# Suaiba/Mammo-CLIP-Dissect

Hardware: AMD Instinct MI355X
Metric: probe images/sec dissected (763 concepts, all layers) (higher is better)
Workload: dtype f32; 1 GPU; configs[1]: M-Mammo-CLIP Dissect through the drop-in driver describe_broad_neurons.main(): Mammo-CLIP ViT-B/16 target+dissector (random init), weak: 10000 images per GPU, synthetic 224x224 images resident in HBM, 763 concepts, 12 layers x 768 neurons, soft_wpmi top_k=100; CSV + args.txt + activation cache files written inside the step; entry_point=mammo_clip_dissect_amd.concept_vit.describe_broad_neurons.main, images_per_gpu=10000, global_images=10000, batch=2500, parallelism=image-sharded dp1, activation_cache_written=True

## Files before the change

mammo-clip-dissect_amd/csrc/k_attn.hip:

```cpp
#include "mcd_common.h"
#include "../../include/mcd_text.h"
#include "../../include/mcd_clip.h"
#include "../../include/mcd_sentence.h"

namespace {

using f32x16 = __attribute__((ext_vector_type(16))) float;

constexpr int AT_D = 64;
constexpr int AT_MAX_T = 256;
constexpr int AT_LONG_MAX_T = 32768;
constexpr int AT_HALF = 32 * 256;
constexpr int AT_STAGE = 2 * AT_HALF;
constexpr int AT_NSTAGE = 4;
constexpr int AT_REL = 2 * AT_MAX_T + 32;

template <bool KEYLEN, bool CAUSAL = false, bool BIAS = false>
__device__ __forceinline__ void attn_block(const float* __restrict__ qkv, int T, int H, int64_t b, int h, int q0, int ncw,
                                           int L, float* __restrict__ out, const float* __restrict__ rel = nullptr) {
    __shared__ __attribute__((aligned(1024))) char at_lds[AT_NSTAGE * AT_STAGE];
    const float* rel_s = nullptr;
    if constexpr (BIAS) {
        __shared__ float at_rel[AT_REL];
        for (int i = threadIdx.x; i < AT_REL; i += blockDim.x) {
            const int d = i - (T - 1);
            at_rel[i] = d < L ? rel[max(d, 1 - L) + T - 1] * 1.44269504088896340736f : 0.f;
        }
        rel_s = at_rel;
        __syncthreads();
    }
    const int TK = KEYLEN ? L : T;
    const int ntile = (TK + 31) >> 5;
    const int64_t row_stride = (int64_t)3 * H * AT_D;
    const float* base = qkv + b * T * row_stride + (int64_t)h * AT_D;
    const int lane = threadIdx.x & 63;
    const int wave = __builtin_amdgcn_readfirstlane(threadIdx.x >> 6);
    const int ql = lane & 31, half = lane >> 5;
    const int q = q0 + wave * 32 + ql;

    if (wave == ncw) {
        auto stage = [&](int kt) {
            __amdgpu_buffer_rsrc_t rs = __builtin_amdgcn_make_buffer_rsrc((void*)(qkv + b * T * row_stride), 0,
                                                                            (int)(T * row_stride * 4), 0x00020000);
            char* dst = at_lds + (kt % AT_NSTAGE) * AT_STAGE;
            const int v_off = H * AT_D * 4;
#pragma unroll
            for (int p = 0; p < 8; ++p) {
                const int r = 4 * p + (lane >> 4);
                const int c = (lane & 15) ^ (r & 15);
                int key = kt * 32 + r;
                if (key >= TK) key = TK - 1;
                const unsigned off = (unsigned)(((int64_t)key * row_stride + (int64_t)(h + H) * AT_D + c * 4) * 4);
                __builtin_amdgcn_raw_ptr_buffer_load_lds(rs, (__attribute__((address_space(3))) void*)(dst + p * 1024), 16, off, 0, 0, 0);
                __builtin_amdgcn_raw_ptr_buffer_load_lds(rs, (__attribute__((address_space(3))) void*)(dst + AT_HALF + p * 1024), 16, off,
                                                         v_off, 0, 0);
            }
        };
        stage(0);
        if (ntile > 1) stage(1);
        for (int kt = 0; kt < ntile; kt += 2) {
            asm volatile("s_waitcnt vmcnt(0)" ::: "memory");
            __builtin_amdgcn_s_barrier();
            asm volatile("" ::: "memory");
            if (kt + 2 < ntile) stage(kt + 2);
            if (kt + 3 < ntile) stage(kt + 3);
        }
        return;
    }

    const float qs = 0.125f * 1.44269504088896340736f;
    float Qr[32];
    const float* qrow = base + (int64_t)(q < T ? q : T - 1) * row_stride + 4 * half;
    float4 qv[8];
#pragma unroll
    for (int j = 0; j < 8; ++j) qv[j] = *reinterpret_cast<const float4*>(qrow + 8 * j);
#pragma unroll
    for (int j = 0; j < 8; ++j) {
        const float4 t = qv[j];
        Qr[4 * j + 0] = t.x * qs;
        Qr[4 * j + 1] = t.y * qs;
        Qr[4 * j + 2] = t.z * qs;
        Qr[4 * j + 3] = t.w * qs;
    }

    const int kx = ql & 15;
    const int k_off = ql * 256;
    const int v_row = 4 * half * 256 + (ql & 3) * 4;
    const int va = (ql >> 2) ^ (half << 2);

    f32x16 o[2];
#pragma unroll
    for (int i = 0; i < 2; ++i)
#pragma unroll
        for (int r = 0; r < 16; ++r) o[i][r] = 0.f;
    float m = -INFINITY, l = 0.f;
    const int rel_q = T - 1 - (q < T ? q : T - 1) + 4 * half;

    const int ntile_w = CAUSAL ? min(ntile, (q0 >> 5) + wave + 1) : ntile;
    for (int kt = 0; kt < ntile_w; ++kt) {
        if ((kt & 1) == 0) __builtin_amdgcn_s_barrier();
        asm volatile("" ::: "memory");
        const char* kb = at_lds + (kt % AT_NSTAGE) * AT_STAGE;
        const char* vb = kb + AT_HALF;
        int kx_t = kx, va_t = va;
        asm volatile("" : "+v"(kx_t), "+v"(va_t));
        int v_off[4];
#pragma unroll
        for (int e = 0; e < 4; ++e) v_off[e] = v_row + ((va_t ^ e) << 4);

        f32x16 c;
#pragma unroll
        for (int r = 0; r < 16; ++r) c[r] = 0.f;
#pragma unroll
        for (int j = 0; j < 8; ++j) {
            const float4 ka = *reinterpret_cast<const float4*>(kb + k_off + (((2 * j + half) ^ kx_t) << 4));
            c = __builtin_amdgcn_mfma_f32_32x32x2f32(ka.x, Qr[4 * j + 0], c, 0, 0, 0);
            c = __builtin_amdgcn_mfma_f32_32x32x2f32(ka.y, Qr[4 * j + 1], c, 0, 0, 0);
            c = __builtin_amdgcn_mfma_f32_32x32x2f32(ka.z, Qr[4 * j + 2], c, 0, 0, 0);
            c = __builtin_amdgcn_mfma_f32_32x32x2f32(ka.w, Qr[4 * j + 3], c, 0, 0, 0);
        }
        if constexpr (BIAS) {
            const float* rb = rel_s + rel_q + kt * 32;
#pragma unroll
            for (int r = 0; r < 16; ++r) c[r] += rb[(r & 3) + 8 * (r >> 2)];
        }
        if constexpr (CAUSAL) {
            if (kt == ntile_w - 1) {
#pragma unroll
                for (int r = 0; r < 16; ++r)
                    if ((r & 3) + 8 * (r >> 2) + 4 * half > ql) c[r] = -INFINITY;
            }
        } else {
            const int nk = TK - kt * 32;
            if (nk < 32) {
#pragma unroll
                for (int r = 0; r < 16; ++r)
                    if ((r & 3) + 8 * (r >> 2) + 4 * half >= nk) c[r] = -INFINITY;
            }
        }
        float mt = c[0];
#pragma unroll
        for (int r = 1; r < 16; ++r) mt = fmaxf(mt, c[r]);
        mt = fmaxf(mt, __shfl_xor(mt, 32));
        const float m_new = fmaxf(m, mt);
        const float alpha = __builtin_amdgcn_exp2f(m - m_new);
        float ls = 0.f;
#pragma unroll
        for (int r = 0; r < 16; ++r) {
            c[r] = __builtin_amdgcn_exp2f(c[r] - m_new);
            ls += c[r];
        }
        l = l * alpha + ls;
        m = m_new;
#pragma unroll
        for (int i = 0; i < 2; ++i)
#pragma unroll
            for (int r = 0; r < 16; ++r) o[i][r] *= alpha;
        auto pv_step = [&](int r) {
            const int k0 = (r & 3) + 8 * (r >> 2);
            const char* vr = vb + k0 * 256 + v_off[r & 3];
            const float v0 = *reinterpret_cast<const float*>(vr + ((0 ^ (k0 & 8)) << 4));
            const float v1 = *reinterpret_cast<const float*>(vr + ((8 ^ (k0 & 8)) << 4));
            o[0] = __builtin_amdgcn_mfma_f32_32x32x2f32(v0, c[r], o[0], 0, 0, 0);
            o[1] = __builtin_amdgcn_mfma_f32_32x32x2f32(v1, c[r], o[1], 0, 0, 0);
        };
#pragma unroll
        for (int r = 0; r < 16; ++r) {
            if ((r & 3) == 0 && r) asm volatile("" ::: "memory");
            pv_step(r);
        }
    }

    l = l + __shfl_xor(l, 32);
    if (q < T) {
        const float inv = 1.0f / l;
        float* dst = out + (b * T + q) * (int64_t)H * AT_D + (int64_t)h * AT_D + 4 * half;
#pragma unroll
        for (int i = 0; i < 2; ++i)
#pragma unroll
            for (int g = 0; g < 4; ++g) {
                const float4 t = make_float4(o[i][4 * g + 0] * inv, o[i][4 * g + 1] * inv, o[i][4 * g + 2] * inv,
                                             o[i][4 * g + 3] * inv);
                *reinterpret_cast<float4*>(dst + 32 * i + 8 * g) = t;
            }
    }
    if constexpr (CAUSAL) {
        for (int kt = (ntile_w + 1) & ~1; kt < ntile; kt += 2) __builtin_amdgcn_s_barrier();
    }
}

__global__ __launch_bounds__(576, 4) void vit_attention_kernel(const float* __restrict__ qkv, int T, int H,
                                                                float* __restrict__ out) {
    const int ntile = (T + 31) >> 5;
    const int h = blockIdx.x;
    const int64_t b = blockIdx.y;
    attn_block<false>(qkv, T, H, b, h, 0, ntile, T, out);
}

__global__ __launch_bounds__(576, 4) void vit_attention_keylen_kernel(const float* __restrict__ qkv, int T, int H,
                                                                       const int32_t* __restrict__ lens,
                                                                       float* __restrict__ out) {
    const int ncw = (T + 31) >> 5;
    const int h = blockIdx.x;
    const int64_t b = blockIdx.y;
    int L = T;
    if (lens) L = min(max(lens[b], 1), T);
    attn_block<true>(qkv, T, H, b, h, 0, ncw, __builtin_amdgcn_readfirstlane(L), out);
}

__global__ __launch_bounds__(576, 4) void vit_attention_relbias_kernel(const float* __restrict__ qkv, int T, int H,
                                                                        const int32_t* __restrict__ lens,
                                                                        const float* __restrict__ rel,
                                                                        float* __restrict__ out) {
    const int ncw = (T + 31) >> 5;
    const int h = blockIdx.x;
    const int64_t b = blockIdx.y;
    int L = T;
    if (lens) L = min(max(lens[b], 1), T);
    attn_block<true, false, true>(qkv, T, H, b, h, 0, ncw, __builtin_amdgcn_readfirstlane(L), out,
                                  rel + (int64_t)h * (2 * T - 1));
}

__global__ __launch_bounds__(576, 4) void vit_attention_causal_kernel(const float* __restrict__ qkv, int T, int H,
                                                                       float* __restrict__ out) {
    const int ntile = (T + 31) >> 5;
    const int h = blockIdx.x;
    const int64_t b = blockIdx.y;
    attn_block<false, true>(qkv, T, H, b, h, 0, ntile, T, out);
}

__global__ __launch_bounds__(576, 4) void vit_attention_long_kernel(const float* __restrict__ qkv, int T, int H, int nqb,
                                                                     int npairs, int per_xcd, float* __restrict__ out) {
    const int pair = (int)(blockIdx.x & 7) * per_xcd + (int)(blockIdx.x >> 3);
    if (pair >= npairs) return;
    const int grp = pair / nqb;
    const int ncw = min(8, (T + 31) >> 5);
    attn_block<false>(qkv, T, H, grp / H, grp % H, (pair - grp * nqb) * 32 * ncw, ncw, T, out);
}

constexpr int AC_WAVES = 4;
constexpr int AC_U = 4;
constexpr int AC_SPLIT_T = 512;
constexpr int AC_MAX_T = 32768;

template <int CTRL>
__device__ __forceinline__ float ac_dpp_add(float x) {
    return x + __builtin_bit_cast(float, __builtin_amdgcn_update_dpp(0, __builtin_bit_cast(int, x), CTRL, 0xf, 0xf, true));
}

__device__ __forceinline__ float ac_row_sum(float x) {
    x = ac_dpp_add<0xB1>(x);
    x = ac_dpp_add<0x4E>(x);
    x = ac_dpp_add<0x141>(x);
    return ac_dpp_add<0x140>(x);
}

__global__ __launch_bounds__(64 * AC_WAVES) void vit_attention_cls_kernel(
    const float* __restrict__ q, int64_t q_img, const float* __restrict__ k, int64_t k_row, int64_t k_img,
    const float* __restrict__ v, int64_t v_row, int64_t v_img, int T, int H, int64_t npairs, int S, float* __restrict__ out) {
    __shared__ float4 st_acc[AC_WAVES * 4][16];
    __shared__ float st_m[AC_WAVES * 4], st_l[AC_WAVES * 4];
    const int lane = threadIdx.x & 63;
    const int wave = __builtin_amdgcn_readfirstlane(threadIdx.x >> 6);
    const int sub = lane & 15, g = lane >> 4;
    const int64_t pair = (int64_t)blockIdx.x * (AC_WAVES / S) + wave / S;
    const int slice = wave % S;
    const bool live = pair < npairs;

    float m = -1e30f, l = 0.f;
    float4 acc = make_float4(0.f, 0.f, 0.f, 0.f);
    if (live) {
        const int64_t b = pair / H;
        const int h = (int)(pair - b * H);
        const float qs = 0.125f * 1.44269504088896340736f;
        float4 qv = *reinterpret_cast<const float4*>(q + b * q_img + (int64_t)h * AT_D + 4 * sub);
        qv.x *= qs; qv.y *= qs; qv.z *= qs; qv.w *= qs;
        const int r0 = slice * 4 + g;
        const float* kp = k + b * k_img + (int64_t)r0 * k_row + (int64_t)h * AT_D + 4 * sub;
        const float* vp = v + b * v_img + (int64_t)r0 * v_row + (int64_t)h * AT_D + 4 * sub;
        const int64_t kstep = (int64_t)4 * S * k_row, vstep = (int64_t)4 * S * v_row;
        for (int rb = slice * 4; rb < T; rb += 4 * S * AC_U) {
            float4 kk[AC_U], vv[AC_U];
            bool ok[AC_U];
#pragma unroll
            for (int u = 0; u < AC_U; ++u) {
                ok[u] = rb + u * 4 * S + g < T;
                kk[u] = make_float4(0.f, 0.f, 0.f, 0.f);
                vv[u] = make_float4(0.f, 0.f, 0.f, 0.f);
                if (ok[u]) {
                    kk[u] = *reinterpret_cast<const float4*>(kp + u * kstep);
                    vv[u] = *reinterpret_cast<const float4*>(vp + u * vstep);
                }
            }
            kp += AC_U * kstep;
            vp += AC_U * vstep;
            float s[AC_U];
            float mt = m;
#pragma unroll
            for (int u = 0; u < AC_U; ++u) {
                const float d = fmaf(kk[u].w, qv.w, fmaf(kk[u].z, qv.z, fmaf(kk[u].y, qv.y, kk[u].x * qv.x)));
                const float r = ac_row_sum(d);
                s[u] = ok[u] ? r : -INFINITY;
                mt = fmaxf(mt, s[u]);
            }
            const float alpha = __builtin_amdgcn_exp2f(m - mt);
            m = mt;
            l *= alpha;
            acc.x *= alpha; acc.y *= alpha; acc.z *= alpha; acc.w *= alpha;
#pragma unroll
            for (int u = 0; u < AC_U; ++u) {
                const float p = __builtin_amdgcn_exp2f(s[u] - mt);
                l += p;
                acc.x = fmaf(p, vv[u].x, acc.x);
                acc.y = fmaf(p, vv[u].y, acc.y);
                acc.z = fmaf(p, vv[u].z, acc.z);
                acc.w = fmaf(p, vv[u].w, acc.w);
            }
        }
    }
    st_acc[wave * 4 + g][sub] = acc;
    if (sub == 0) {
        st_m[wave * 4 + g] = m;
        st_l[wave * 4 + g] = l;
    }
    __syncthreads();
    if (live && slice == 0) {
        const int s0 = wave * 4, ns = 4 * S;
        float mx = st_m[s0];
        for (int i = 1; i < ns; ++i) mx = fmaxf(mx, st_m[s0 + i]);
        float num = 0.f, den = 0.f;
        const float* accf = reinterpret_cast<const float*>(&st_acc[s0][0]);
        for (int i = 0; i < ns; ++i) {
            const float w = __builtin_amdgcn_exp2f(st_m[s0 + i] - mx);
            num = fmaf(accf[i * 64 + lane], w, num);
            den = fmaf(st_l[s0 + i], w, den);
        }
        out[pair * AT_D + lane] = num / den;
    }
}

}

extern "C" int mcd_vit_attention(const float* qkv, int64_t B, int64_t T, int64_t H, float* out, mcd_stream_t stream) {
    MCD_REQUIRE(qkv && out, MCD_E_ARG, "mcd_vit_attention: NULL pointer");
    MCD_REQUIRE(B >= 0 && T >= 1 && H >= 1, MCD_E_ARG, "mcd_vit_attention: bad shape B=%lld T=%lld H=%lld", (long long)B,
                (long long)T, (long long)H);
    MCD_REQUIRE(T <= AT_MAX_T, MCD_E_UNSUPPORTED, "mcd_vit_attention: T=%lld tokens, at most %d (one wave per 32 queries, 8 waves)",
                (long long)T, AT_MAX_T);
    MCD_REQUIRE(B <= 65535 && H <= 65535, MCD_E_UNSUPPORTED, "mcd_vit_attention: B and H must be <= 65535");
    MCD_REQUIRE(((uintptr_t)qkv) % 16 == 0 && ((uintptr_t)out) % 16 == 0, MCD_E_ARG,
                "mcd_vit_attention: qkv and out must be 16-byte aligned");
    if (B == 0) return MCD_OK;
    const int nwaves = (int)((T + 31) / 32) + 1;
    hipLaunchKernelGGL(vit_attention_kernel, dim3((unsigned)H, (unsigned)B), dim3(64 * nwaves), 0, (hipStream_t)stream, qkv,
                       (int)T, (int)H, out);
    MCD_LAUNCH_CHECK("vit_attention_kernel");
    return MCD_OK;
}

extern "C" int mcd_vit_attention_keylen(const float* qkv, int64_t B, int64_t T, int64_t H, const int32_t* lens, float* out,
                                        mcd_stream_t stream) {
    MCD_REQUIRE(qkv && out, MCD_E_ARG, "mcd_vit_attention_keylen: NULL pointer");
    MCD_REQUIRE(B >= 0 && T >= 1 && H >= 1, MCD_E_ARG, "mcd_vit_attention_keylen: bad shape B=%lld T=%lld H=%lld",
                (long long)B, (long long)T, (long long)H);
    MCD_REQUIRE(T <= AT_MAX_T, MCD_E_UNSUPPORTED,
                "mcd_vit_attention_keylen: T=%lld tokens, at most %d (one wave per 32 queries, 8 waves)", (long long)T, AT_MAX_T);
    MCD_REQUIRE(B <= 65535 && H <= 65535, MCD_E_UNSUPPORTED, "mcd_vit_attention_keylen: B and H must be <= 65535");
    MCD_REQUIRE(((uintptr_t)qkv) % 16 == 0 && ((uintptr_t)out) % 16 == 0 && ((uintptr_t)lens) % 4 == 0, MCD_E_ARG,
                "mcd_vit_attention_keylen: qkv and out must be 16-byte aligned, lens 4-byte aligned");
    if (B == 0) return MCD_OK;
    const int nwaves = (int)((T + 31) / 32) + 1;
    hipLaunchKernelGGL(vit_attention_keylen_kernel, dim3((unsigned)H, (unsigned)B), dim3(64 * nwaves), 0, (hipStream_t)stream,
                       qkv, (int)T, (int)H, lens, out);
    MCD_LAUNCH_CHECK("vit_attention_keylen_kernel");
    return MCD_OK;
}

extern "C" int mcd_vit_attention_relbias(const float* qkv, int64_t B, int64_t T, int64_t H, const int32_t* lens,
                                         const float* rel, float* out, mcd_stream_t stream) {
    MCD_REQUIRE(qkv && out, MCD_E_ARG, "mcd_vit_attention_relbias: NULL pointer");
    MCD_REQUIRE(B >= 0 && T >= 1 && H >= 1, MCD_E_ARG, "mcd_vit_attention_relbias: bad shape B=%lld T=%lld H=%lld",
                (long long)B, (long long)T, (long long)H);
    MCD_REQUIRE(T <= AT_MAX_T, MCD_E_UNSUPPORTED,
                "mcd_vit_attention_relbias: T=%lld tokens, at most %d (one wave per 32 queries, 8 waves)", (long long)T, AT_MAX_T);
    MCD_REQUIRE(B <= 65535 && H <= 65535, MCD_E_UNSUPPORTED, "mcd_vit_attention_relbias: B and H must be <= 65535");
    MCD_REQUIRE(((uintptr_t)qkv) % 16 == 0 && ((uintptr_t)out) % 16 == 0 && ((uintptr_t)lens) % 4 == 0 &&
                    ((uintptr_t)rel) % 16 == 0,
                MCD_E_ARG, "mcd_vit_attention_relbias: qkv, out and rel must be 16-byte aligned, lens 4-byte aligned");
    if (B == 0) return MCD_OK;
    const int nwaves = (int)((T + 31) / 32) + 1;
    if (!rel) {
        hipLaunchKernelGGL(vit_attention_keylen_kernel, dim3((unsigned)H, (unsigned)B), dim3(64 * nwaves), 0,
                           (hipStream_t)stream, qkv, (int)T, (int)H, lens, out);
        MCD_LAUNCH_CHECK("vit_attention_keylen_kernel");
        return MCD_OK;
    }
    hipLaunchKernelGGL(vit_attention_relbias_kernel, dim3((unsigned)H, (unsigned)B), dim3(64 * nwaves), 0, (hipStream_t)stream,
                       qkv, (int)T, (int)H, lens, rel, out);
    MCD_LAUNCH_CHECK("vit_attention_relbias_kernel");
    return MCD_OK;
}

extern "C" int mcd_vit_attention_causal(const float* qkv, int64_t B, int64_t T, int64_t H, float* out, mcd_stream_t stream) {
    MCD_REQUIRE(qkv && out, MCD_E_ARG, "mcd_vit_attention_causal: NULL pointer");
    MCD_REQUIRE(B >= 0 && T >= 1 && H >= 1, MCD_E_ARG, "mcd_vit_attention_causal: bad shape B=%lld T=%lld H=%lld", (long long)B,
                (long long)T, (long long)H);
    MCD_REQUIRE(T <= AT_MAX_T, MCD_E_UNSUPPORTED,
                "mcd_vit_attention_causal: T=%lld tokens, at most %d (one wave per 32 queries, 8 waves)", (long long)T, AT_MAX_T);
    MCD_REQUIRE(B <= 65535 && H <= 65535, MCD_E_UNSUPPORTED, "mcd_vit_attention_causal: B and H must be <= 65535");
    MCD_REQUIRE(((uintptr_t)qkv) % 16 == 0 && ((uintptr_t)out) % 16 == 0, MCD_E_ARG,
                "mcd_vit_attention_causal: qkv and out must be 16-byte aligned");
    if (B == 0) return MCD_OK;
    const int nwaves = (int)((T + 31) / 32) + 1;
    hipLaunchKernelGGL(vit_attention_causal_kernel, dim3((unsigned)H, (unsigned)B), dim3(64 * nwaves), 0, (hipStream_t)stream,
                       qkv, (int)T, (int)H, out);
    MCD_LAUNCH_CHECK("vit_attention_causal_kernel");
    return MCD_OK;
}

extern "C" int mcd_vit_attention_long(const float* qkv, int64_t B, int64_t T, int64_t H, float* out, mcd_stream_t stream) {
    MCD_REQUIRE(qkv && out, MCD_E_ARG, "mcd_vit_attention_long: NULL pointer");
    MCD_REQUIRE(B >= 0 && T >= 1 && H >= 1, MCD_E_ARG, "mcd_vit_attention_long: bad shape B=%lld T=%lld H=%lld",
                (long long)B, (long long)T, (long long)H);
    MCD_REQUIRE(T <= AT_LONG_MAX_T, MCD_E_UNSUPPORTED, "mcd_vit_attention_long: T=%lld tokens, at most %d", (long long)T,
                AT_LONG_MAX_T);
    MCD_REQUIRE(B <= INT32_MAX && H <= 65535, MCD_E_UNSUPPORTED, "mcd_vit_attention_long: B must be < 2^31, H <= 65535");
    MCD_REQUIRE(T * 3 * H * AT_D * 4 <= INT32_MAX, MCD_E_UNSUPPORTED,
                "mcd_vit_attention_long: one image's qkv block (T=%lld x H=%lld heads) must stay under 2^31 bytes",
                (long long)T, (long long)H);
    MCD_REQUIRE(((uintptr_t)qkv) % 16 == 0 && ((uintptr_t)out) % 16 == 0, MCD_E_ARG,
                "mcd_vit_attention_long: qkv and out must be 16-byte aligned");
    if (B == 0) return MCD_OK;
    const int64_t ncw = std::min<int64_t>(8, (T + 31) / 32);
    const int64_t nqb = mcd_cdiv((T + 31) / 32, ncw);
    const int64_t npairs = B * H * nqb;
    MCD_REQUIRE(npairs <= INT32_MAX / 576 - 8, MCD_E_UNSUPPORTED,
                "mcd_vit_attention_long: B=%lld x H=%lld x %lld query blocks is too large a grid", (long long)B,
                (long long)H, (long long)nqb);
    const int64_t per_xcd = mcd_cdiv(npairs, 8);
    hipLaunchKernelGGL(vit_attention_long_kernel, dim3((unsigned)(8 * per_xcd)), dim3(64 * (unsigned)(ncw + 1)), 0,
                       (hipStream_t)stream, qkv, (int)T, (int)H, (int)nqb, (int)npairs, (int)per_xcd, out);
    MCD_LAUNCH_CHECK("vit_attention_long_kernel");
    return MCD_OK;
}

extern "C" int mcd_vit_attention_cls(const float* q, int64_t q_img, const float* k, int64_t k_row, int64_t k_img,
                                     const float* v, int64_t v_row, int64_t v_img, int64_t B, int64_t T, int64_t H,
                                     float* out, mcd_stream_t stream) {
    MCD_REQUIRE(q && k && v && out, MCD_E_ARG, "mcd_vit_attention_cls: NULL pointer");
    MCD_REQUIRE(B >= 0 && T >= 1 && H >= 1, MCD_E_ARG, "mcd_vit_attention_cls: bad shape B=%lld T=%lld H=%lld", (long long)B,
                (long long)T, (long long)H);
    MCD_REQUIRE(T <= AC_MAX_T, MCD_E_UNSUPPORTED, "mcd_vit_attention_cls: T=%lld tokens, at most %d", (long long)T, AC_MAX_T);
    MCD_REQUIRE(H <= 65535 && B <= INT32_MAX / 65535, MCD_E_UNSUPPORTED,
                "mcd_vit_attention_cls: H must be <= 65535 and B * 65535 < 2^31");
    const int64_t W = H * AT_D;
    MCD_REQUIRE(q_img >= W && k_row >= W && v_row >= W && k_img >= W && v_img >= W, MCD_E_ARG,
                "mcd_vit_attention_cls: a stride (q_img=%lld k_row=%lld k_img=%lld v_row=%lld v_img=%lld) is below H*64=%lld",
                (long long)q_img, (long long)k_row, (long long)k_img, (long long)v_row, (long long)v_img, (long long)W);
    MCD_REQUIRE(((uintptr_t)q) % 16 == 0 && ((uintptr_t)k) % 16 == 0 && ((uintptr_t)v) % 16 == 0 && ((uintptr_t)out) % 16 == 0 &&
                    q_img % 4 == 0 && k_row % 4 == 0 && k_img % 4 == 0 && v_row % 4 == 0 && v_img % 4 == 0,
                MCD_E_ARG, "mcd_vit_attention_cls: pointers must be 16-byte aligned and strides multiples of 4 floats");
    if (B == 0) return MCD_OK;
    const int S = T > AC_SPLIT_T ? AC_WAVES : 1;
    const int64_t npairs = B * H;
    const int64_t nwg = mcd_cdiv(npairs, (int64_t)(AC_WAVES / S));
    hipLaunchKernelGGL(vit_attention_cls_kernel, dim3((unsigned)nwg), dim3(64 * AC_WAVES), 0, (hipStream_t)stream, q, q_img, k,
                       k_row, k_img, v, v_row, v_img, (int)T, (int)H, npairs, S, out);
    MCD_LAUNCH_CHECK("vit_attention_cls_kernel");
    return MCD_OK;
}
```

Baseline: 4102 images/s.

## Rework attention MFMA tiling from 32x32x2 to 16x16x4 with sub-tile masking

Replaces the per-wave 32x32x2 f32 MFMA attention inner loop with 16x16x4 MFMAs, splitting each wave's 32 queries into two 16-row groups and keys into 16-key subtiles. Tail and causal subtiles are skipped at compile-time granularity, and row max/sum reductions use permlane16/32 swaps instead of shuffles. This aims to cut wasted MFMA work on partial tiles (ViT T=197 leaves a ragged last tile) and raise matrix throughput per instruction. It increases code complexity, register pressure (two accumulator sets, templated tile variants) and swizzle addressing risk.

```diff
diff --git a/mammo-clip-dissect_amd/csrc/k_attn.hip b/mammo-clip-dissect_amd/csrc/k_attn.hip
--- a/mammo-clip-dissect_amd/csrc/k_attn.hip
+++ b/mammo-clip-dissect_amd/csrc/k_attn.hip
@@ -5,7 +5,7 @@
 
 namespace {
 
-using f32x16 = __attribute__((ext_vector_type(16))) float;
+using f32x4 = __attribute__((ext_vector_type(4))) float;
 
 constexpr int AT_D = 64;
 constexpr int AT_MAX_T = 256;
@@ -14,6 +14,22 @@
 constexpr int AT_STAGE = 2 * AT_HALF;
 constexpr int AT_NSTAGE = 4;
 constexpr int AT_REL = 2 * AT_MAX_T + 32;
+
+template <typename F>
+__device__ __forceinline__ float at_groups_reduce(float x, F op) {
+    const unsigned xb = __builtin_bit_cast(unsigned, x);
+    auto s = __builtin_amdgcn_permlane16_swap(xb, xb, false, false);
+    x = op(__builtin_bit_cast(float, (unsigned)s[0]), __builtin_bit_cast(float, (unsigned)s[1]));
+    const unsigned yb = __builtin_bit_cast(unsigned, x);
+    s = __builtin_amdgcn_permlane32_swap(yb, yb, false, false);
+    return op(__builtin_bit_cast(float, (unsigned)s[0]), __builtin_bit_cast(float, (unsigned)s[1]));
+}
+__device__ __forceinline__ float at_groups_max(float x) {
+    return at_groups_reduce(x, [](float a, float b) { return fmaxf(a, b); });
+}
+__device__ __forceinline__ float at_groups_sum(float x) {
+    return at_groups_reduce(x, [](float a, float b) { return a + b; });
+}
 
 template <bool KEYLEN, bool CAUSAL = false, bool BIAS = false>
 __device__ __forceinline__ void attn_block(const float* __restrict__ qkv, int T, int H, int64_t b, int h, int q0, int ncw,
@@ -35,8 +51,7 @@
     const float* base = qkv + b * T * row_stride + (int64_t)h * AT_D;
     const int lane = threadIdx.x & 63;
     const int wave = __builtin_amdgcn_readfirstlane(threadIdx.x >> 6);
-    const int ql = lane & 31, half = lane >> 5;
-    const int q = q0 + wave * 32 + ql;
+    const int n = lane & 15, g = lane >> 4;
 
     if (wave == ncw) {
         auto stage = [&](int kt) {
@@ -68,125 +83,181 @@
         return;
     }
 
+    const int qw = q0 + wave * 32;
+    const int nsub = (TK + 15) >> 4;
+    const int ns0 = qw < T ? (CAUSAL ? min(nsub, (qw >> 4) + 1) : nsub) : 0;
+    const int ns1 = qw + 16 < T ? (CAUSAL ? min(nsub, (qw >> 4) + 2) : nsub) : 0;
+
     const float qs = 0.125f * 1.44269504088896340736f;
-    float Qr[32];
-    const float* qrow = base + (int64_t)(q < T ? q : T - 1) * row_stride + 4 * half;
-    float4 qv[8];
-#pragma unroll
-    for (int j = 0; j < 8; ++j) qv[j] = *reinterpret_cast<const float4*>(qrow + 8 * j);
-#pragma unroll
-    for (int j = 0; j < 8; ++j) {
-        const float4 t = qv[j];
-        Qr[4 * j + 0] = t.x * qs;
-        Qr[4 * j + 1] = t.y * qs;
-        Qr[4 * j + 2] = t.z * qs;
-        Qr[4 * j + 3] = t.w * qs;
-    }
-
-    const int kx = ql & 15;
-    const int k_off = ql * 256;
-    const int v_row = 4 * half * 256 + (ql & 3) * 4;
-    const int va = (ql >> 2) ^ (half << 2);
-
-    f32x16 o[2];
-#pragma unroll
-    for (int i = 0; i < 2; ++i)
-#pragma unroll
-        for (int r = 0; r < 16; ++r) o[i][r] = 0.f;
-    float m = -INFINITY, l = 0.f;
-    const int rel_q = T - 1 - (q < T ? q : T - 1) + 4 * half;
-
-    const int ntile_w = CAUSAL ? min(ntile, (q0 >> 5) + wave + 1) : ntile;
-    for (int kt = 0; kt < ntile_w; ++kt) {
+    float Q[2][16];
+    {
+        float4 qv[2][4];
+#pragma unroll
+        for (int j = 0; j < 2; ++j) {
+            const float* qrow = base + (int64_t)min(qw + 16 * j + n, T - 1) * row_stride + 16 * g;
+#pragma unroll
+            for (int c = 0; c < 4; ++c) qv[j][c] = *reinterpret_cast<const float4*>(qrow + 4 * c);
+        }
+#pragma unroll
+        for (int j = 0; j < 2; ++j)
+#pragma unroll
+            for (int c = 0; c < 4; ++c) {
+                Q[j][4 * c + 0] = qv[j][c].x * qs;
+                Q[j][4 * c + 1] = qv[j][c].y * qs;
+                Q[j][4 * c + 2] = qv[j][c].z * qs;
+                Q[j][4 * c + 3] = qv[j][c].w * qs;
+            }
+    }
+
+    const int kg = ((4 - g) & 3) * 4;
+    const int k_row = ((4 - (n >> 2)) & 3) * 4 + (n & 3);
+    const int k_base = k_row * 256 + (((4 * g) ^ k_row) << 4);
+    const int v_base = kg * 256 + ((n ^ kg) << 4);
+
+    f32x4 o[2][4];
+#pragma unroll
+    for (int j = 0; j < 2; ++j)
+#pragma unroll
+        for (int i = 0; i < 4; ++i)
+#pragma unroll
+            for (int r = 0; r < 4; ++r) o[j][i][r] = 0.f;
+    float m[2] = {-INFINITY, -INFINITY}, l[2] = {0.f, 0.f};
+    const int nsw[2] = {ns0, ns1};
+    const int kg_n = kg - n;
+    const int rel_q[2] = {T - 1 - min(qw + n, T - 1) + kg, T - 1 - min(qw + 16 + n, T - 1) + kg};
+
+    auto tile = [&](auto ns0_c, auto ns1_c, int kt) {
+        constexpr int NS[2] = {decltype(ns0_c)::value, decltype(ns1_c)::value};
+        constexpr int NSM = NS[0] > NS[1] ? NS[0] : NS[1];
         if ((kt & 1) == 0) __builtin_amdgcn_s_barrier();
         asm volatile("" ::: "memory");
         const char* kb = at_lds + (kt % AT_NSTAGE) * AT_STAGE;
         const char* vb = kb + AT_HALF;
-        int kx_t = kx, va_t = va;
-        asm volatile("" : "+v"(kx_t), "+v"(va_t));
-        int v_off[4];
-#pragma unroll
-        for (int e = 0; e < 4; ++e) v_off[e] = v_row + ((va_t ^ e) << 4);
-
-        f32x16 c;
-#pragma unroll
-        for (int r = 0; r < 16; ++r) c[r] = 0.f;
-#pragma unroll
-        for (int j = 0; j < 8; ++j) {
-            const float4 ka = *reinterpret_cast<const float4*>(kb + k_off + (((2 * j + half) ^ kx_t) << 4));
-            c = __builtin_amdgcn_mfma_f32_32x32x2f32(ka.x, Qr[4 * j + 0], c, 0, 0, 0);
-            c = __builtin_amdgcn_mfma_f32_32x32x2f32(ka.y, Qr[4 * j + 1], c, 0, 0, 0);
-            c = __builtin_amdgcn_mfma_f32_32x32x2f32(ka.z, Qr[4 * j + 2], c, 0, 0, 0);
-            c = __builtin_amdgcn_mfma_f32_32x32x2f32(ka.w, Qr[4 * j + 3], c, 0, 0, 0);
-        }
-        if constexpr (BIAS) {
-            const float* rb = rel_s + rel_q + kt * 32;
-#pragma unroll
-            for (int r = 0; r < 16; ++r) c[r] += rb[(r & 3) + 8 * (r >> 2)];
-        }
-        if constexpr (CAUSAL) {
-            if (kt == ntile_w - 1) {
-#pragma unroll
-                for (int r = 0; r < 16; ++r)
-                    if ((r & 3) + 8 * (r >> 2) + 4 * half > ql) c[r] = -INFINITY;
-            }
-        } else {
-            const int nk = TK - kt * 32;
-            if (nk < 32) {
-#pragma unroll
-                for (int r = 0; r < 16; ++r)
-                    if ((r & 3) + 8 * (r >> 2) + 4 * half >= nk) c[r] = -INFINITY;
-            }
-        }
-        float mt = c[0];
-#pragma unroll
-        for (int r = 1; r < 16; ++r) mt = fmaxf(mt, c[r]);
-        mt = fmaxf(mt, __shfl_xor(mt, 32));
-        const float m_new = fmaxf(m, mt);
-        const float alpha = __builtin_amdgcn_exp2f(m - m_new);
-        float ls = 0.f;
-#pragma unroll
-        for (int r = 0; r < 16; ++r) {
-            c[r] = __builtin_amdgcn_exp2f(c[r] - m_new);
-            ls += c[r];
-        }
-        l = l * alpha + ls;
-        m = m_new;
-#pragma unroll
-        for (int i = 0; i < 2; ++i)
-#pragma unroll
-            for (int r = 0; r < 16; ++r) o[i][r] *= alpha;
-        auto pv_step = [&](int r) {
-            const int k0 = (r & 3) + 8 * (r >> 2);
-            const char* vr = vb + k0 * 256 + v_off[r & 3];
-            const float v0 = *reinterpret_cast<const float*>(vr + ((0 ^ (k0 & 8)) << 4));
-            const float v1 = *reinterpret_cast<const float*>(vr + ((8 ^ (k0 & 8)) << 4));
-            o[0] = __builtin_amdgcn_mfma_f32_32x32x2f32(v0, c[r], o[0], 0, 0, 0);
-            o[1] = __builtin_amdgcn_mfma_f32_32x32x2f32(v1, c[r], o[1], 0, 0, 0);
-        };
-#pragma unroll
-        for (int r = 0; r < 16; ++r) {
-            if ((r & 3) == 0 && r) asm volatile("" ::: "memory");
-            pv_step(r);
-        }
-    }
-
-    l = l + __shfl_xor(l, 32);
-    if (q < T) {
-        const float inv = 1.0f / l;
-        float* dst = out + (b * T + q) * (int64_t)H * AT_D + (int64_t)h * AT_D + 4 * half;
-#pragma unroll
-        for (int i = 0; i < 2; ++i)
-#pragma unroll
-            for (int g = 0; g < 4; ++g) {
-                const float4 t = make_float4(o[i][4 * g + 0] * inv, o[i][4 * g + 1] * inv, o[i][4 * g + 2] * inv,
-                                             o[i][4 * g + 3] * inv);
-                *reinterpret_cast<float4*>(dst + 32 * i + 8 * g) = t;
-            }
-    }
-    if constexpr (CAUSAL) {
-        for (int kt = (ntile_w + 1) & ~1; kt < ntile; kt += 2) __builtin_amdgcn_s_barrier();
-    }
+        int k_t = k_base, v_t = v_base;
+        asm volatile("" : "+v"(k_t), "+v"(v_t));
+
+        f32x4 c[2][2];
+#pragma unroll
+        for (int j = 0; j < 2; ++j) {
+            int ri = BIAS ? rel_q[j] + kt * 32 : 0;
+            if constexpr (BIAS) asm volatile("" : "+v"(ri));
+#pragma unroll
+            for (int u = 0; u < 2; ++u)
+#pragma unroll
+                for (int r = 0; r < 4; ++r) {
+                    c[j][u][r] = 0.f;
+                    if constexpr (BIAS)
+                        if (u < NS[j]) c[j][u][r] = rel_s[ri + 16 * u + r];
+                }
+        }
+#pragma unroll
+        for (int cc = 0; cc < 4; ++cc) {
+            float ka[NSM][4];
+#pragma unroll
+            for (int u = 0; u < NSM; ++u) {
+                const float4 t = *reinterpret_cast<const float4*>(kb + u * 4096 + (k_t ^ (cc << 4)));
+                ka[u][0] = t.x; ka[u][1] = t.y; ka[u][2] = t.z; ka[u][3] = t.w;
+            }
+#pragma unroll
+            for (int e = 0; e < 4; ++e)
+#pragma unroll
+                for (int u = 0; u < NSM; ++u)
+#pragma unroll
+                    for (int j = 0; j < 2; ++j)
+                        if (u < NS[j]) c[j][u] = __builtin_amdgcn_mfma_f32_16x16x4f32(ka[u][e], Q[j][4 * cc + e], c[j][u], 0, 0, 0);
+        }
+
+#pragma unroll
+        for (int j = 0; j < 2; ++j) {
+            if (NS[j] == 0) continue;
+            if constexpr (CAUSAL) {
+                if (kt == ((nsw[j] - 1) >> 1)) {
+#pragma unroll
+                    for (int u = 0; u < NS[j]; ++u)
+#pragma unroll
+                        for (int r = 0; r < 4; ++r)
+                            if (kg_n > qw + 16 * j - kt * 32 - 16 * u - r) c[j][u][r] = -INFINITY;
+                }
+            } else {
+                const int nk = TK - kt * 32;
+                if (nk < 16 * NS[j]) {
+#pragma unroll
+                    for (int u = 0; u < NS[j]; ++u)
+#pragma unroll
+                        for (int r = 0; r < 4; ++r)
+                            if (16 * u + kg + r >= nk) c[j][u][r] = -INFINITY;
+                }
+            }
+            float mt = c[j][0][0];
+#pragma unroll
+            for (int u = 0; u < NS[j]; ++u)
+#pragma unroll
+                for (int r = 0; r < 4; ++r)
+                    if (u || r) mt = fmaxf(mt, c[j][u][r]);
+            mt = at_groups_max(mt);
+            const float m_new = fmaxf(m[j], mt);
+            const float alpha = __builtin_amdgcn_exp2f(m[j] - m_new);
+            float ls = 0.f;
+#pragma unroll
+            for (int u = 0; u < NS[j]; ++u)
+#pragma unroll
+                for (int r = 0; r < 4; ++r) {
+                    c[j][u][r] = __builtin_amdgcn_exp2f(c[j][u][r] - m_new);
+                    ls += c[j][u][r];
+                }
+            l[j] = l[j] * alpha + ls;
+            m[j] = m_new;
+#pragma unroll
+            for (int i = 0; i < 4; ++i)
+#pragma unroll
+                for (int r = 0; r < 4; ++r) o[j][i][r] *= alpha;
+        }
+
+#pragma unroll
+        for (int u = 0; u < NSM; ++u)
+#pragma unroll
+            for (int r = 0; r < 4; ++r) {
+                const float4 t = *reinterpret_cast<const float4*>(vb + u * 4096 + r * 256 + (v_t ^ (r << 4)));
+                const float vf[4] = {t.x, t.y, t.z, t.w};
+#pragma unroll
+                for (int i = 0; i < 4; ++i)
+#pragma unroll
+                    for (int j = 0; j < 2; ++j)
+                        if (u < NS[j]) o[j][i] = __builtin_amdgcn_mfma_f32_16x16x4f32(vf[i], c[j][u][r], o[j][i], 0, 0, 0);
+            }
+    };
+
+    using I0 = std::integral_constant<int, 0>;
+    using I1 = std::integral_constant<int, 1>;
+    using I2 = std::integral_constant<int, 2>;
+    if (ns1 == 0) {
+        for (int kt = 0; kt < (ns0 >> 1); ++kt) tile(I2{}, I0{}, kt);
+        if (ns0 & 1) tile(I1{}, I0{}, ns0 >> 1);
+    } else {
+        for (int kt = 0; kt < (ns0 >> 1); ++kt) tile(I2{}, I2{}, kt);
+        if (ns0 & 1) {
+            if constexpr (CAUSAL) tile(I1{}, I2{}, ns0 >> 1);
+            else tile(I1{}, I1{}, ns0 >> 1);
+        }
+    }
+
+    int tid = threadIdx.x;
+    asm volatile("" : "+v"(tid));
+#pragma unroll
+    for (int j = 0; j < 2; ++j) {
+        const float lt = at_groups_sum(l[j]);
+        const int q = qw + 16 * j + (tid & 15);
+        if (nsw[j] > 0 && q < T) {
+            const float inv = 1.0f / lt;
+            float* dst = out + (b * T + q) * (int64_t)H * AT_D + (int64_t)h * AT_D + ((tid >> 4) & 3) * 16;
+#pragma unroll
+            for (int r = 0; r < 4; ++r)
+                *reinterpret_cast<float4*>(dst + 4 * r) =
+                    make_float4(o[j][0][r] * inv, o[j][1][r] * inv, o[j][2][r] * inv, o[j][3][r] * inv);
+        }
+    }
+    const int nt_w = (max(ns0, ns1) + 1) >> 1;
+    for (int kt = (nt_w + 1) & ~1; kt < ntile; kt += 2) __builtin_amdgcn_s_barrier();
 }
 
 __global__ __launch_bounds__(576, 4) void vit_attention_kernel(const float* __restrict__ qkv, int T, int H,
```

Result: no change. 4119 images/s (median of 6 runs) (+0.4%).
